# aexoden/snesimage

Hardware: AMD Instinct MI355X
Metric: candidate palettes scored/sec (higher is better)
Workload: dtype f32

## Files before the change

snesimage_amd/csrc/capi.hip:

```cpp
#include "../../include/snesimage_hip.h"
#include "kernels.hpp"
#include "kernels_opt.hpp"
#include "kernels_fast.hpp"
#include "kernels_sparse.hpp"
#include "kernels_sparse2.hpp"
#include "kernels_batch.hpp"
#include "kernels_shared.hpp"
#include "kernels_tile.hpp"

#include <hip/hip_runtime.h>

#include <atomic>
#include <cmath>
#include <cstdio>
#include <cstdlib>
#include <cstring>
#include <string>
#include <utility>
#include <memory>
#include <vector>

using namespace snes;

namespace {
// ... 114 lines not shown
        uint32_t h2q_max = 512;
        bool down_tiles = true;
        uint32_t h0_min = 1024;
        bool base_down_side = false;
        uint32_t h0_grid = 8192;
        hipStream_t h0_stream[8] = {}; hipEvent_t ev_scan[8] = {}, ev_h0[8] = {}, ev_hn[8] = {}, ev_vn[8] = {};
        bool v0_aside = true;
        hipEvent_t ev_v0[8] = {};
        bool vn_aside = true;
        uint32_t tiles_grid = 4096;
        uint32_t down1_grid = 32768;
        bool vsplit = true;
        uint32_t scan4_max = 2048;
        uint32_t hgrid = 8192;
        bool dedup = true; uint32_t dedup_min = 1024; int *holder = nullptr; bool holder_dirty = false;
        bool enabled = false, side = true; uint32_t min_n = 1; uint32_t cap = 0, lanes = 0;
        SparseGeom S{};
        float *store = nullptr, *cand_tab = nullptr, *cand_lab = nullptr, *ckf = nullptr, *ckh = nullptr; long long zeros_off = 0; uint32_t *bitmap = nullptr; double *cka = nullptr, *part = nullptr;
        CandMeta *meta = nullptr; unsigned int *items = nullptr; int *item_count = nullptr; long long item_stride = 0; int *order = nullptr, *first = nullptr;
        uint4 *plist = nullptr; int *plist_count = nullptr; bool plist_valid = false;
        hipStream_t base_stream = nullptr; hipEvent_t ev_base_in = nullptr, ev_base_h = nullptr, ev_base_done = nullptr, ev_base_narrow = nullptr;
        uint8_t *dmaps = nullptr, *dmapsC4 = nullptr;
        uint8_t *bmap = nullptr, *bmapC4 = nullptr, *bcand = nullptr; unsigned long long *dpack = nullptr; double *ckd = nullptr; uint32_t slot_ci = 0;
        float *rec_lab = nullptr;
        int base_sp = -1, base_si = -1;
        struct Ahead { uint8_t *bmap = nullptr, *bmapC4 = nullptr, *bcand = nullptr; unsigned long long *dpack = nullptr; double *ckd = nullptr; float *btab = nullptr, *blab = nullptr, *rec_lab = nullptr; int *ok = nullptr;
                       hipEvent_t ev = nullptr; bool on = true, have = false; int sp = -1, si = -1; unsigned long long epoch = 0; } ahead;
    } sp;
    uint8_t *d_cand = nullptr; uint32_t cand_cap = 0;
    uint8_t *d_cand_sel = nullptr;
// ... 296 lines not shown
    HIPCHK(dmalloc(&sp.store, sizeof(float) * (size_t)S.cand_stride * ncap));
    if (g_poison_alloc.load()) HIPCHK(hipMemsetAsync(sp.store, 0xff, sizeof(float) * (size_t)S.cand_stride * ncap, c->stream));
    HIPCHK(dmalloc(&sp.cand_tab, sizeof(float) * 8 * ncap));
    if (c->perceptual) {
        dfree(sp.cand_lab); dfree(sp.bitmap);
        HIPCHK(dmalloc(&sp.cand_lab, sizeof(float) * 3 * ncap));
        HIPCHK(dmalloc(&sp.bitmap, sizeof(uint32_t) * (c->npx / 32) * ncap));
    }
    HIPCHK(dmalloc(&sp.ckf, sizeof(float) * (size_t)okf));
    dfree(sp.ckh); HIPCHK(dmalloc(&sp.ckh, sizeof(float) * (size_t)(okh + 12LL * G.W + 256)));
    sp.zeros_off = okh;
    HIPCHK(hipMemsetAsync(sp.ckh + okh, 0, sizeof(float) * 12 * (size_t)G.W, c->stream));
    HIPCHK(dmalloc(&sp.cka, sizeof(double) * (size_t)oka));
    HIPCHK(dmalloc(&sp.part, sizeof(double) * ncap * kMaxScales * 18));
    HIPCHK(dmalloc(&sp.meta, sizeof(CandMeta) * ncap));
    dfree(sp.order); HIPCHK(dmalloc(&sp.order, sizeof(int) * ncap));
    dfree(sp.first); HIPCHK(dmalloc(&sp.first, sizeof(int) * ncap));
    HIPCHK(dmalloc(&sp.items, sizeof(unsigned int) * (size_t)sp.item_stride * kItemLists * (c->nlanes + 1)));
    if (!sp.base_stream && sp.side) {
        int prio_lo = 0, prio_hi = 0;
        HIPCHK(hipDeviceGetStreamPriorityRange(&prio_lo, &prio_hi));
        HIPCHK(hipStreamCreateWithPriority(&sp.base_stream, hipStreamNonBlocking, prio_hi));
        HIPCHK(hipEventCreateWithFlags(&sp.ev_base_in, hipEventDisableTiming));
        HIPCHK(hipEventCreateWithFlags(&sp.ev_base_h, hipEventDisableTiming));
        HIPCHK(hipEventCreateWithFlags(&sp.ev_base_narrow, hipEventDisableTiming));
        HIPCHK(hipEventCreateWithFlags(&sp.ev_base_done, hipEventDisableTiming));
    }
    HIPCHK(dmalloc(&sp.item_count, sizeof(int) * (kItemLists * (c->nlanes + 1) + 1)));
    HIPCHK(hipMemsetAsync(sp.item_count, 0, sizeof(int) * (kItemLists * (c->nlanes + 1) + 1), c->stream));
    sp.plist_count = sp.item_count + (size_t)kItemLists * (c->nlanes + 1);
    sp.counters_cleared = true;
// ... 171 lines not shown
        else if (c->ditherw && c->sub_size == 15) hipLaunchKernelGGL((k_ditherw<15>), dim3((nc + 3) / 4), dim3(256), 0, stream, Dp, (int)nc);
        else if (c->ditherw && c->sub_size > 1) hipLaunchKernelGGL((k_ditherw<0>), dim3((nc + 3) / 4), dim3(256), 0, stream, Dp, (int)nc);
        else if (c->sub_size == 15) hipLaunchKernelGGL((k_dither<false, 15, 2>), dim3(nc), dim3(128), 0, stream, Dp);
        else hipLaunchKernelGGL((k_dither<false, 0, 2>), dim3(nc), dim3(128), 0, stream, Dp);
        hipLaunchKernelGGL(k_dither_diff, dim3((nc + 3) / 4), dim3(1024), 0, stream, P);
    } else if (c->perceptual) {
        hipLaunchKernelGGL(k_candidate_lab, dim3((nc + 63) / 64), dim3(64), 0, stream, sp.cand_tab + 8 * (size_t)P.k0, (int)nc, c->d_lab_eotf, sp.cand_lab + 3 * (size_t)P.k0);
        HIPCHK(hipMemsetAsync(sp.bitmap + (size_t)P.k0 * (c->npx / 32), 0, sizeof(uint32_t) * (c->npx / 32) * nc, stream));
        hipLaunchKernelGGL(k_sparse_scan_lab, dim3(nc), dim3(256), 0, stream, P);
    } else if (nc <= sp.scan4_max) hipLaunchKernelGGL(k_sparse_scan4, dim3((nc + 3) / 4), dim3(1024), 0, stream, P);
    else hipLaunchKernelGGL(k_sparse_scan, dim3((nc + 15) / 16), dim3(1024), 0, stream, P);
    bool vn_aside = false;
    const bool h0_ahead = sp.side && sp.h0_min > 0 && nc >= sp.h0_min && nc > sp.h2q_max && lane < 8 && P.s_first > 0;
    const bool v0_aside = h0_ahead && sp.v0_aside;
    vn_aside = h0_ahead && !v0_aside && sp.vn_aside && P.s_first < G.nscales;
    if (c->sp.lpt && nc > 512) P.order = sp.order + P.k0;
    if (h0_ahead) {
        if (!sp.h0_stream[lane]) {
            HIPCHK(hipStreamCreateWithFlags(&sp.h0_stream[lane], hipStreamNonBlocking));
            HIPCHK(hipEventCreateWithFlags(&sp.ev_scan[lane], hipEventDisableTiming));
            HIPCHK(hipEventCreateWithFlags(&sp.ev_h0[lane], hipEventDisableTiming));
            HIPCHK(hipEventCreateWithFlags(&sp.ev_hn[lane], hipEventDisableTiming));
            HIPCHK(hipEventCreateWithFlags(&sp.ev_v0[lane], hipEventDisableTiming));
            HIPCHK(hipEventCreateWithFlags(&sp.ev_vn[lane], hipEventDisableTiming));
        }
        hipStream_t hs = sp.h0_stream[lane];
        HIPCHK(hipEventRecord(sp.ev_scan[lane], stream));
        HIPCHK(hipStreamWaitEvent(hs, sp.ev_scan[lane], 0));
        HIPCHK(hipStreamWaitEvent(hs, sp.ev_base_h, 0));
        size_t gx = ((size_t)nc * (G.sh[0] / 4) * 3 + 15) / 16; if (gx > sp.h0_grid) gx = sp.h0_grid;
        hipLaunchKernelGGL(k_sparse_h2, dim3((unsigned)gx, (unsigned)kColBuckets), dim3(64), h2_lds(c), hs, P);
// ... 34 lines not shown
    if (sp.side || stream != c->stream) HIPCHK(hipStreamWaitEvent(stream, sp.side ? sp.ev_base_done : c->ev_ready, 0));
    if (c->sp.lpt && nc > 512) {
        if (!h0_ahead) hipLaunchKernelGGL(k_sparse_order, dim3(1), dim3(1024), 0, stream, P, sp.order + P.k0);
        P.order = sp.order + P.k0;
    }
    if (vn_aside) {
        hipStream_t hs = sp.h0_stream[lane];
        HIPCHK(hipStreamWaitEvent(hs, sp.ev_hn[lane], 0));
        HIPCHK(hipStreamWaitEvent(hs, sp.ev_base_narrow, 0));
        hipLaunchKernelGGL(k_sparse_v, dim3((nc * 3 + 7) / 8, (unsigned)(G.nscales - P.s_first)), dim3(256), 0, hs, P);
        HIPCHK(hipEventRecord(sp.ev_vn[lane], hs));
    }
    if (v0_aside) {
        if (sp.side) HIPCHK(hipStreamWaitEvent(stream, sp.ev_base_narrow, 0));
        if (P.s_first < G.nscales) hipLaunchKernelGGL(k_sparse_v, dim3((nc * 3 + 7) / 8, (unsigned)(G.nscales - P.s_first)), dim3(256), 0, stream, P);
        if (P.s_first > 1) hipLaunchKernelGGL(k_sparse_v2_from, dim3(nc * 3, (unsigned)(P.s_first - 1)), dim3(256), 0, stream, P, 1);
    } else {
    if (c->timing) HIPCHK(hipEventRecord(tr.ev[3], stream));
    hipLaunchKernelGGL(k_sparse_v2, dim3(nc * 3, (unsigned)P.s_first), dim3(256), 0, stream, P);
    if (c->timing) HIPCHK(hipEventRecord(tr.ev[4], stream));
    }
    if (vn_aside) HIPCHK(hipStreamWaitEvent(stream, sp.ev_vn[lane], 0));
    else if (!v0_aside) {
    if (sp.side) HIPCHK(hipStreamWaitEvent(stream, sp.ev_base_narrow, 0));
    if (P.s_first < G.nscales) hipLaunchKernelGGL(k_sparse_v, dim3((nc * 3 + 7) / 8, (unsigned)(G.nscales - P.s_first)), dim3(256), 0, stream, P);
    }
    if (v0_aside) HIPCHK(hipStreamWaitEvent(stream, sp.ev_v0[lane], 0));
    hipLaunchKernelGGL(k_final_score_wave, dim3((nc + 3) / 4), dim3(256), 0, stream, sp.part + (size_t)P.k0 * G.nscales * 18, (int)nc, G, d_errors, err_stride, err_offset, P.item_count, (int)kItemLists);
    if (c->dither) {
        uint8_t *bm = lane == 0 ? c->d_bestmap : c->extra[lane - 1].d_bestmap; BestRec *br = lane == 0 ? c->d_bestrec : c->extra[lane - 1].d_bestrec;
        hipLaunchKernelGGL(k_keep_best, dim3(1), dim3(1024), 0, stream, d_errors, err_stride, err_offset, (int)nc, P.maps, (int)c->npx, br, bm);
    }
    HIPCHK(hipGetLastError());
    if (c->timing) { tr.light = c->timing != 1; if (!tr.light) HIPCHK(hipEventRecord(tr.ev[5], stream)); c->t_pending.push_back(tr); }
    return SNES_OK;
}

struct LaneScope {
    snesimage_ctx *c; snesimage_ctx::Lane *L;
    LaneScope(snesimage_ctx *c_, snesimage_ctx::Lane *L_) : c(c_), L(L_) { swap(); }
    ~LaneScope() { swap(); }
    void swap() { std::swap(c->stream, L->stream); std::swap(c->d_work, L->d_work); std::swap(c->d_cand_tab, L->d_cand_tab); std::swap(c->d_cand_lab, L->d_cand_lab);
                  std::swap(c->d_part, L->d_part); std::swap(c->d_maps, L->d_maps); std::swap(c->d_mapsT, L->d_mapsT); std::swap(c->d_mapsC4, L->d_mapsC4); std::swap(c->d_mapsR4, L->d_mapsR4);
// ... 212 lines not shown
    if (const char *e = getenv("SNES_DITHER_REC")) c->dither_rec = atoi(e) != 0;
    if (const char *e = getenv("SNES_DITHER4_MAX")) { int v = atoi(e); if (v >= 0) c->dither4_max = (uint32_t)v; }
    if (const char *e = getenv("SNES_DOWN1_GRID")) { int v = atoi(e); if (v >= 64) c->sp.down1_grid = (uint32_t)v; }
    if (const char *e = getenv("SNES_VSPLIT")) c->sp.vsplit = atoi(e) != 0;
    if (const char *e = getenv("SNES_DOWN_TILES")) c->sp.down_tiles = atoi(e) != 0;
    if (const char *e = getenv("SNES_V0_ASIDE")) c->sp.v0_aside = atoi(e) != 0;
    if (const char *e = getenv("SNES_VN_ASIDE")) c->sp.vn_aside = atoi(e) != 0;
    if (const char *e = getenv("SNES_H0_GRID")) { int v = atoi(e); if (v >= 16) c->sp.h0_grid = (uint32_t)v; }
    if (const char *e = getenv("SNES_H0_MIN")) { int v = atoi(e); if (v >= 0) c->sp.h0_min = (uint32_t)v; }
    if (const char *e = getenv("SNES_TILES_GRID")) { int v = atoi(e); if (v >= 64) c->sp.tiles_grid = (uint32_t)v; }
    if (const char *e = getenv("SNES_SCAN4_MAX")) { int v = atoi(e); if (v >= 0) c->sp.scan4_max = (uint32_t)v; }
    if (const char *e = getenv("SNES_H2Q_MAX")) { int v = atoi(e); if (v >= 0) c->sp.h2q_max = (uint32_t)v; }
    if (const char *e = getenv("SNES_HGRID")) { int v = atoi(e); if (v >= 1) c->sp.hgrid = (uint32_t)v; }
    if (const char *e = getenv("SNES_SPARSE_MIN")) { int v = atoi(e); if (v >= 1) c->sp.min_n = (uint32_t)v; }
    if (const char *e = getenv("SNES_DEDUP")) c->sp.dedup = atoi(e) != 0;
    if (const char *e = getenv("SNES_DEDUP_MIN")) { int v = atoi(e); if (v >= 1) c->sp.dedup_min = (uint32_t)v; }
    Geom &G = c->G;
    G.W = (int)w; G.H = (int)h; G.nscales = 0;
    int P2 = 8;
    while (P2 < (int)h) P2 *= 2;
    for (int s = 0; s < kMaxScales; s++) {
        if (s > 0 && (G.sw[s - 1] < 8 || G.th[s - 1] < 8)) break;
        G.sw[s] = (int)w >> s; G.th[s] = s == 0 ? (int)h : (G.th[s - 1] + 1) / 2; G.sh[s] = s == 0 ? (int)h : P2 >> s; G.nscales = s + 1;
    }
    long long off = 0, soff = 0;
    for (int s = 0; s < G.nscales; s++) {
        long long N = (long long)G.sw[s] * G.sh[s];
        G.src_off[s] = soff; soff += 3 * N;
        if (s >= 1) { G.off_xyb[s] = off; off += 3 * N; G.off_xybT[s] = off; off += 3 * N; } else { G.off_xyb[s] = 0; G.off_xybT[s] = 0; }
        G.off_hout[s] = off; off += 9 * N;
// ... 60 lines not shown
}

void batch_forget(struct snesimage_batch *b, snesimage_ctx *c);
void group_forget(struct snesimage_group *g, snesimage_ctx *c);
namespace { void window_free(struct snesimage_window *w); void tile_free(snesimage_ctx *c); }
void snesimage_destroy(snesimage_ctx *c) {
    if (!c) return;
    (void)hipSetDevice(c->device);
    if (c->tile) { if (c->stream) (void)hipStreamSynchronize(c->stream); tile_free(c); }
    if (c->win) { if (c->stream) (void)hipStreamSynchronize(c->stream); window_free(c->win); c->win = nullptr; }
    if (c->owner) batch_forget(c->owner, c);
    if (c->group) group_forget(c->group, c);
    if (c->ev_own) (void)hipEventDestroy(c->ev_own);
    if (c->stream) (void)hipStreamSynchronize(c->stream);
    (void)drain_timing(c);
    dfree(c->d_packC4); dfree(c->d_packR4); dfree(c->d_subC4); dfree(c->d_subR4); dfree(c->d_mapsC4); dfree(c->d_mapsR4); dfree(c->d_img1C4); dfree(c->d_mu1R4); dfree(c->d_sd1R4); dfree(c->d_r1); dfree(c->d_r1R4); dfree(c->d_a1); dfree(c->d_a1R4);
    dfree(c->d_orig); dfree(c->d_tile_pal); dfree(c->d_colors); dfree(c->d_map); dfree(c->d_pack); dfree(c->d_packT); dfree(c->d_eotf); dfree(c->d_lab_eotf);
    dfree(c->d_pal_rgb8); dfree(c->d_pal_lin); dfree(c->d_pal_xyb); dfree(c->d_pal_lab); dfree(c->d_lin0); dfree(c->d_img1); dfree(c->d_img1T); dfree(c->d_mu1); dfree(c->d_sd1);
    dfree(c->d_bestmaps_all); dfree(c->d_bestrecs_all); dfree(c->d_skip); dfree(c->d_rplist); dfree(c->d_rcount); dfree(c->d_rtab); dfree(c->d_rlab); dfree(c->d_tile_cost); dfree(c->d_tile_any); dfree(c->d_tile_moved);
    dfree(c->d_labpx); dfree(c->d_labpxT); dfree(c->d_work); dfree(c->d_cand_tab); dfree(c->d_cand_lab); dfree(c->d_part); dfree(c->d_maps); dfree(c->d_mapsT);
    dfree(c->d_cand); dfree(c->d_cand_sel); dfree(c->d_errs); dfree(c->d_errs_sel); dfree(c->d_inc_err); dfree(c->d_last); dfree(c->d_scratch_err); dfree(c->d_dummy_cand);
    for (auto &L : c->extra) { if (L.stream) (void)hipStreamSynchronize(L.stream); dfree(L.d_mapsC4); dfree(L.d_mapsR4); dfree(L.d_work); dfree(L.d_cand_tab); dfree(L.d_cand_lab); dfree(L.d_part); dfree(L.d_maps); dfree(L.d_mapsT); if (L.done) (void)hipEventDestroy(L.done); if (L.stream) (void)hipStreamDestroy(L.stream); }
    if (c->ev_ready) (void)hipEventDestroy(c->ev_ready);
    { auto &q = c->sp; for (int i = 0; i < 8; i++) if (q.h0_stream[i]) { (void)hipStreamSynchronize(q.h0_stream[i]); (void)hipStreamDestroy(q.h0_stream[i]); (void)hipEventDestroy(q.ev_scan[i]); (void)hipEventDestroy(q.ev_h0[i]); (void)hipEventDestroy(q.ev_hn[i]); (void)hipEventDestroy(q.ev_vn[i]); (void)hipEventDestroy(q.ev_v0[i]); }
      if (q.base_stream) { (void)hipStreamSynchronize(q.base_stream); (void)hipStreamDestroy(q.base_stream); (void)hipEventDestroy(q.ev_base_in); (void)hipEventDestroy(q.ev_base_h); (void)hipEventDestroy(q.ev_base_narrow); (void)hipEventDestroy(q.ev_base_done); } dfree(q.store); dfree(q.cand_tab); dfree(q.ckf); dfree(q.cka); dfree(q.part); dfree(q.meta); dfree(q.items); dfree(q.item_count); dfree(q.plist); dfree(q.order); dfree(q.first); dfree(q.holder); dfree(q.cand_lab); dfree(q.bitmap); dfree(q.ckh);
      dfree(q.dmaps); dfree(q.dmapsC4); dfree(q.bmap); dfree(q.bmapC4); dfree(q.bcand); dfree(q.dpack); dfree(q.ckd);
      dfree(q.rec_lab); dfree(q.ahead.blab); dfree(q.ahead.rec_lab); dfree(q.ahead.bmap); dfree(q.ahead.bmapC4); dfree(q.ahead.bcand); dfree(q.ahead.dpack); dfree(q.ahead.ckd); dfree(q.ahead.btab); dfree(q.ahead.ok); if (q.ahead.ev) (void)hipEventDestroy(q.ahead.ev); }
    kmeans_free(c->km);
    if (c->own_stream) (void)hipStreamDestroy(c->own_stream);
    delete c;
// ... 397 lines not shown
```

snesimage_amd/csrc/kernels.hpp:

```cpp
#pragma once
#include "color.hpp"

namespace snes {

constexpr int kMaxScales = SSIM2_NUM_SCALES;
constexpr int kBlurRadius = 5;

SNES_HD long long idx_c4(int x, int y, int H) { return ((long long)(x >> 2) * H + y) * 4 + (x & 3); }
SNES_HD long long idx_r4(int x, int y, int W) { return ((long long)(y >> 2) * W + x) * 4 + (y & 3); }
SNES_HD long long idx_xt4(int x, int y, int H) { return ((((long long)(x >> 6) * (H >> 2)) + (y >> 2)) << 8) + ((x & 63) << 2) + (y & 3); }

struct BlurK {
    float n2[3];
    float d1[3];
};

struct Geom {
    int W, H, nscales;
    int sw[kMaxScales], sh[kMaxScales];
    int th[kMaxScales];
    long long off_xyb[kMaxScales], off_xybT[kMaxScales], off_hout[kMaxScales];
    long long cand_stride;
    long long src_off[kMaxScales];
};
// ... 647 lines not shown
                ssim = fma(kSsim2Weight[i], fabs(avg_edge[n]), ssim); i++;
                ssim = fma(kSsim2Weight[i], fabs(avg_edge[n + 2]), ssim); i++;
            }
        }
    ssim *= SSIM2_SCORE_SCALE;
    ssim = fma(SSIM2_SCORE_C3 * ssim * ssim, ssim, fma(SSIM2_SCORE_C1, ssim, SSIM2_SCORE_C2 * ssim * ssim));
    if (ssim > 0.0) ssim = fma(pow(ssim, SSIM2_SCORE_EXP), SSIM2_SCORE_GAIN, SSIM2_SCORE_MAX);
    else ssim = SSIM2_SCORE_MAX;
    errors[(size_t)err_offset + (size_t)c * err_stride] = 100.0 - ssim;
}

__device__ __forceinline__ double readlane_f64(double v, int l) {
    const int lo = __builtin_amdgcn_readlane(__double2loint(v), l), hi = __builtin_amdgcn_readlane(__double2hiint(v), l);
    return __hiloint2double(hi, lo);
}
__device__ __forceinline__ void final_score_wave_body(const double *__restrict__ part, int ncand, const Geom &G, double *__restrict__ errors, int err_stride, int err_offset, int *__restrict__ zero, int nzero) {
    const int gt = blockIdx.x * blockDim.x + threadIdx.x;
    if (zero && gt < nzero) zero[gt] = 0;
    const int lane = threadIdx.x & 63, c = __builtin_amdgcn_readfirstlane(gt >> 6);
    if (c >= ncand) return;
    const int ns = G.nscales, npair = 3 * ns;
    double term[6] = {0.0, 0.0, 0.0, 0.0, 0.0, 0.0};
    if (lane < npair) {
        const int ch = lane / ns, s = lane - ch * ns;
        const double *p = part + (((size_t)c * ns + s) * 3 + ch) * 6;
        const double opp = 1.0 / (double)((size_t)G.sw[s] * G.th[s]);
        term[0] = opp * p[0]; term[1] = opp * p[2]; term[2] = opp * p[4];
        term[3] = sqrt(sqrt(opp * p[1])); term[4] = sqrt(sqrt(opp * p[3])); term[5] = sqrt(sqrt(opp * p[5]));
    }
    double ssim = 0.0;
    int i = 0;
    for (int l = 0; l < npair; l++) {
#pragma unroll
        for (int t = 0; t < 6; t++) { ssim = fma(kSsim2Weight[i], fabs(readlane_f64(term[t], l)), ssim); i++; }
    }
    if (lane != 0) return;
    ssim *= SSIM2_SCORE_SCALE;
    ssim = fma(SSIM2_SCORE_C3 * ssim * ssim, ssim, fma(SSIM2_SCORE_C1, ssim, SSIM2_SCORE_C2 * ssim * ssim));
    if (ssim > 0.0) ssim = fma(pow(ssim, SSIM2_SCORE_EXP), SSIM2_SCORE_GAIN, SSIM2_SCORE_MAX);
    else ssim = SSIM2_SCORE_MAX;
    errors[(size_t)err_offset + (size_t)c * err_stride] = 100.0 - ssim;
}

__global__ void k_candidate_tables(const uint8_t *__restrict__ rgb5, int n, const float *__restrict__ eotf, float *__restrict__ cand_tab) { candidate_tables_body(rgb5, n, eotf, cand_tab); }
__global__ void k_candidate_tables_mark(const uint8_t *__restrict__ rgb5, int n, const float *__restrict__ eotf, float *__restrict__ cand_tab, int *__restrict__ holder, int list0) { candidate_tables_mark_body(rgb5, n, eotf, cand_tab, holder, list0); }
__global__ __launch_bounds__(1024) void k_dedup_copy(const uint8_t *__restrict__ rgb5, int n, int *__restrict__ holder, double *__restrict__ errors, int err_stride, int err_offset) { dedup_copy_body(rgb5, n, holder, errors, err_stride, err_offset); }
__global__ __launch_bounds__(256) void k_prep(PrepParams P) { prep_body(P); }
__global__ void k_final_score(const double *__restrict__ part, int ncand, Geom G, double *__restrict__ errors, int err_stride, int err_offset, int *__restrict__ zero = nullptr, int nzero = 0) {
    final_score_body(part, ncand, G, errors, err_stride, err_offset, zero, nzero);
}
__global__ __launch_bounds__(256) void k_final_score_wave(const double *__restrict__ part, int ncand, Geom G, double *__restrict__ errors, int err_stride, int err_offset, int *__restrict__ zero = nullptr, int nzero = 0) {
    final_score_wave_body(part, ncand, G, errors, err_stride, err_offset, zero, nzero);
}

}
```

snesimage_amd/csrc/kernels_sparse.hpp:

```cpp
#pragma once
#include "kernels.hpp"

namespace snes {

constexpr int kGroupsTotal = 126;

struct CandMeta {
    int ngroups[kMaxScales];
    int xmin;
    int won;
    unsigned char glist[kGroupsTotal + 2];
    short gslot[kGroupsTotal];
    unsigned char gcb[kGroupsTotal];
};
__device__ __forceinline__ int item_k(unsigned int it) { return (int)(it >> 14); }
__device__ __forceinline__ int item_g(unsigned int it) { return (int)((it >> 8) & 63u); }
__device__ __forceinline__ int item_j(unsigned int it) { return (int)((it >> 2) & 63u); }
__device__ __forceinline__ int item_ch(unsigned int it) { return (int)(it & 3u); }
constexpr int kColBuckets = 4;
constexpr int kItemLists = kMaxScales * kColBuckets;

struct SparseGeom {
    long long off_lin[kMaxScales], off_xybC[kMaxScales], off_xybR[kMaxScales], off_hout[kMaxScales];
    long long cand_stride;
// ... 8 lines not shown
    const unsigned long long *pack, *packC4, *packR4;
    const uint4 *plist; const int *plist_count;
    const float *pal_lin, *pal_xyb, *cand_tab;
    int perceptual; const float *labpx, *cand_lab; uint32_t *bitmap;
    const float *img1C4, *mu1R4, *sd1R4, *a1R4; const double *r1R4;
    float *store; CandMeta *meta;
    unsigned int *items; int *item_count; long long item_stride;
    float *ckf; double *cka; double *part; float *ckh;
    const float *zeros;
    float *trash;
    int use_maps, sub_size; uint32_t slot_ci; const uint8_t *maps, *mapsC4, *bmap, *bmapC4, *subC4, *tile_pal;
    int s_first;
    int *first;
    const int *order;
    const int *holder; int list0;
};

__device__ __forceinline__ uint32_t sparse_ci(uint32_t lo, uint32_t thr, uint32_t crgb, uint32_t ncol) {
    return red_mean_key(crgb, lo & 0x00ffffffu) < thr ? ncol : (lo >> 24);
}

__device__ __forceinline__ uint32_t won_bit(const uint32_t *bm, int px) { return (bm[px >> 5] >> (px & 31)) & 1u; }
__device__ __forceinline__ uint32_t maps_ci(const SparseParams &P, const uint8_t *map, bool is_base, int x0, int y0, uint32_t pack_lo) {
    uint32_t ci = pack_lo >> 24;
    if (ci != (uint32_t)P.ncol + 1u) {
        ci = (uint32_t)P.tile_pal[(x0 >> 3) + (y0 >> 3) * (P.G.W >> 3)] * (uint32_t)P.sub_size + map[y0 * P.G.W + x0];
        if (!is_base && ci == P.slot_ci) ci = (uint32_t)P.ncol;
    }
    return ci;
}

// ... 852 lines not shown
__device__ __forceinline__ void sparse_v_body(const SparseParams &P, const int s) {
    __shared__ float s_lut[256];
    __shared__ short s_gslot[256];
    __shared__ __attribute__((aligned(16))) unsigned char s_raw[(2 + 3) * 3 * 256 * sizeof(float2)];
    float2 (*s_xy)[3][256] = reinterpret_cast<float2 (*)[3][256]>(s_raw);
    float2 (*s_zw)[3][256] = reinterpret_cast<float2 (*)[3][256]>(s_raw + 2 * 3 * 256 * sizeof(float2));
    double (*red)[6] = reinterpret_cast<double (*)[6]>(s_raw);
    static_assert(sizeof(s_raw) >= 256 * 6 * sizeof(double), "reduction scratch must fit the tail ring");
    const Geom &G = P.G;
    if (s >= G.nscales) return;
    const int W = G.sw[s], H = G.sh[s];
    const bool S0 = S0M == 2 ? s == 0 : S0M == 1;
    const int t = threadIdx.x;
    const int ppw = 256 / W;
    const bool is_base = BM == 2 ? P.is_base != 0 : BM == 1;
    const int npairs = is_base ? 3 : P.ncand * 3;
    if ((int)blockIdx.x * ppw >= npairs) return;
    const int ql = t / W, x = t - ql * W;
    const int pair_raw = blockIdx.x * ppw + ql;
    const bool active = pair_raw < npairs;
    const int pair = active ? pair_raw : 0;
    const int k = is_base ? P.base : P.k0 + (P.order ? P.order[pair / 3] : pair / 3), ch = pair % 3;
    if (S0) {
        s_lut[t] = (t < P.ncol + 2) ? P.pal_xyb[3 * t + ch] : 0.0f;
    }
    const size_t ns = (size_t)W * H;
    const int H4 = H >> 2;
    const CandMeta *M = P.meta + k;
    for (int i = t; i < ppw * H4; i += 256) {
        const int pr = blockIdx.x * ppw + i / H4;
        const int pq = (pr < npairs ? pr : 0) / 3;
// ... 258 lines not shown
            queued -= 64;
            if (lane < queued) { const uint32_t v = q[64 + lane]; q[lane] = v; }
        }
    }
    if (lane < queued) full_test((int)q[lane]);
}

__device__ __forceinline__ void sparse_order_body(const SparseParams &P, int *__restrict__ order) {
    __shared__ int s_cnt[66];
    const int t = threadIdx.x, H4 = P.G.sh[0] >> 2;
    const int *first = P.first + P.k0;
    if (t < 66) s_cnt[t] = 0;
    __syncthreads();
    for (int i = t; i < P.ncand; i += blockDim.x) atomicAdd(&s_cnt[first[i]], 1);
    __syncthreads();
    if (t == 0) { int run = 0; for (int b = 0; b <= H4; b++) { const int c = s_cnt[b]; s_cnt[b] = run; run += c; } }
    __syncthreads();
    for (int i = t; i < P.ncand; i += blockDim.x) order[atomicAdd(&s_cnt[first[i]], 1)] = i;
}
__global__ __launch_bounds__(1024) void k_sparse_order(SparseParams P, int *__restrict__ order) { sparse_order_body(P, order); }

__global__ __launch_bounds__(256) void k_sparse_scan_lab(SparseParams P) { sparse_scan_lab_body(P); }
__global__ __launch_bounds__(1024) void k_sparse_scan(SparseParams P) { sparse_scan_body<1>(P); }
__global__ __launch_bounds__(1024) void k_sparse_scan4(SparseParams P) { sparse_scan_body<4>(P); }
__global__ __launch_bounds__(1024) void k_dither_first(SparseParams P) { dither_first_body(P); }
__global__ __launch_bounds__(256) void k_dither_first_lab(SparseParams P) { dither_first_lab_body(P); }
__global__ __launch_bounds__(1024) void k_dither_diff(SparseParams P) { dither_diff_body(P); }
__global__ __launch_bounds__(256) void k_sparse_down(SparseParams P, int only_scale) { sparse_down_body(P, only_scale, (int)blockIdx.x); }
__global__ __launch_bounds__(256) void k_sparse_down1(SparseParams P) { sparse_down1_body(P, (int)blockIdx.x, (int)gridDim.x); }
__global__ __launch_bounds__(256) void k_sparse_down_tiles(SparseParams P) { sparse_down_tiles_body<SNES_DOWN_TILES_U>(P, (int)blockIdx.x, (int)gridDim.x); }
__global__ __launch_bounds__(256) void k_base_down(SparseParams P) { base_down_body(P); }
// ... 6 lines not shown
```

snesimage_amd/csrc/kernels_sparse2.hpp:

```cpp
#pragma once
#include "kernels_sparse.hpp"
#include "kernels_fast.hpp"

namespace snes {

#define SNES_HSTEP(SUM, A, B, OUT)                                                   \
    {                                                                                \
        float o1_ = (SUM) * n2_0, o3_ = (SUM) * n2_1, o5_ = (SUM) * n2_2;            \
        o1_ = fmaf(-1.0f, B[0], o1_); o3_ = fmaf(-1.0f, B[1], o3_); o5_ = fmaf(-1.0f, B[2], o5_); \
        o1_ = fmaf(mp_0, A[0], o1_); o3_ = fmaf(mp_1, A[1], o3_); o5_ = fmaf(mp_2, A[2], o5_);    \
        B[0] = o1_; B[1] = o3_; B[2] = o5_;                                          \
        OUT = o1_ + o3_ + o5_;                                                       \
    }
#define SNES_VSTEP(SUM, A, B, OUT)                                                   \
    {                                                                                \
        float o1_ = fmaf(A[0], d1_0, B[0]), o3_ = fmaf(A[1], d1_1, B[1]), o5_ = fmaf(A[2], d1_2, B[2]); \
        o1_ = fmaf((SUM), n2_0, -o1_); o3_ = fmaf((SUM), n2_1, -o3_); o5_ = fmaf((SUM), n2_2, -o5_);    \
        B[0] = o1_; B[1] = o3_; B[2] = o5_;                                          \
        OUT = o1_ + o3_ + o5_;                                                       \
    }

struct H2Shared {
    __attribute__((aligned(16))) float out[16 * (4 * 32 + 4)];
    long long hbase[16], xbase[16];
// ... 325 lines not shown
    const u32x4 v = __builtin_amdgcn_raw_buffer_load_b128(r, (int)voff, (int)soff, 0);
    return make_double2(__hiloint2double((int)v.y, (int)v.x), __hiloint2double((int)v.w, (int)v.z));
}

template <bool BASE>
__device__ __forceinline__ void sparse_v2_body(const SparseParams &P, const int s, const int bx) {
    __shared__ short s_slot[4][64];
    __shared__ __attribute__((aligned(16))) unsigned char s_raw[(2 + 3) * 3 * 256 * sizeof(float2)];
    double (*red)[6] = reinterpret_cast<double (*)[6]>(s_raw);
    static_assert(sizeof(s_raw) >= 256 * 6 * sizeof(double), "reduction scratch must fit the tail ring");
    const Geom &G = P.G;
    const int W = uni(G.sw[s]), H = uni(G.sh[s]), H4 = H >> 2;
    const int t = threadIdx.x, lane = t & 63;
    const int wv = uni(t >> 6);
    const int wpp = W >> 6, ppw = 4 / wpp;
    const int npairs = BASE ? 3 : P.ncand * 3;
    if (bx * ppw >= npairs) return;
    const int ql = wv / wpp, xw = (wv - ql * wpp) << 6;
    const int pair_raw = bx * ppw + ql;
    const bool active = pair_raw < npairs;
    const int pair = active ? pair_raw : 0;
    const int ch = BASE ? pair : pair / P.ncand, ci = BASE ? 0 : pair - ch * P.ncand;
    const int k = BASE ? P.base : uni(P.k0 + (P.order ? P.order[ci] : ci));
    const CandMeta *M = P.meta + k;
    int gs;
    {
        const int g = lane;
        short sl = -1;
        if (!BASE && g < H4) { sl = M->gslot[P.S.goff[s] + g]; if (sl >= 0 && ((int)M->gcb[P.S.goff[s] + g] << 6) > xw) sl = -1; }
        s_slot[wv][lane] = sl;
        const unsigned long long own = __ballot(sl >= 0);
        gs = BASE ? 0 : uni(own ? __ffsll((long long)own) - 1 : H4 + 1);
    }
    __syncthreads();

    const size_t ns = (size_t)W * H;
    const float *store_k = P.store + (size_t)k * P.S.cand_stride, *store_b = P.store + (size_t)P.base * P.S.cand_stride;
// ... 235 lines not shown

template <bool BASE>
__device__ __forceinline__ void sparse_h2_dispatch(const SparseParams &P, const int list, const int bx, const int gx) {
    const int s = list / kColBuckets;
    if (s >= P.G.nscales || P.G.sw[s] < 64 || (list % kColBuckets) >= (P.G.sw[s] >> 6)) return;
    __shared__ H2Shared sh;
    if (s == 0) sparse_h2_body<true, BASE>(P, list, bx, gx, sh); else sparse_h2_body<false, BASE>(P, list, bx, gx, sh);
}
__global__ __launch_bounds__(64) void k_sparse_h2(SparseParams P) { sparse_h2_dispatch<false>(P, (int)blockIdx.y, (int)blockIdx.x, (int)gridDim.x); }
__global__ __launch_bounds__(64) void k_sparse_h2_from(SparseParams P, int list0) { sparse_h2_dispatch<false>(P, list0 + (int)blockIdx.y, (int)blockIdx.x, (int)gridDim.x); }
__global__ __launch_bounds__(64) void k_sparse_h2q(SparseParams P) { sparse_h2q_dispatch<false>(P, (int)blockIdx.y, (int)blockIdx.x, (int)gridDim.x); }
__global__ __launch_bounds__(64) void k_sparse_h2q_base(SparseParams P) { sparse_h2q_dispatch<true>(P, (int)blockIdx.y, (int)blockIdx.x, (int)gridDim.x); }
__global__ __launch_bounds__(64) void k_sparse_h2_base(SparseParams P) { sparse_h2_dispatch<true>(P, (int)blockIdx.y, (int)blockIdx.x, (int)gridDim.x); }
__global__ __launch_bounds__(256, 5) void k_sparse_v2(SparseParams P) { if ((int)blockIdx.y < P.G.nscales && P.G.sw[blockIdx.y] >= 64) sparse_v2_body<false>(P, (int)blockIdx.y, (int)blockIdx.x); }
__global__ __launch_bounds__(256, 5) void k_sparse_v2_from(SparseParams P, int s0) { const int s = s0 + (int)blockIdx.y; if (s < P.G.nscales && P.G.sw[s] >= 64) sparse_v2_body<false>(P, s, (int)blockIdx.x); }
__global__ __launch_bounds__(128) void k_sparse_v2_base_split(SparseParams P) { const int s = (int)blockIdx.z; if (s < P.G.nscales && P.G.sw[s] >= 64 && (int)blockIdx.x < (P.G.sw[s] >> 6)) sparse_v2_base_split_body(P, s, (int)blockIdx.y, (int)blockIdx.x); }
__global__ __launch_bounds__(256) void k_sparse_v2_base(SparseParams P) { if ((int)blockIdx.y < P.G.nscales && P.G.sw[blockIdx.y] >= 64) sparse_v2_body<true>(P, (int)blockIdx.y, (int)blockIdx.x); }
__device__ __forceinline__ void sparse_v_base_narrow_dispatch(const SparseParams &P) { const int s = (int)blockIdx.y + P.s_first; if (s < P.G.nscales) sparse_v_body<false, 0, 1>(P, s); }
__global__ __launch_bounds__(256, 1) void k_sparse_v_base_narrow(SparseParams P) { sparse_v_base_narrow_dispatch(P); }

}
```

Before: 2.846 million.

## Skip scoring of empty candidates and flatten v2 launch across scales

The LPT ordering kernel now records how many candidates touch any pixels (n_live). The vertical sparse kernels then only process that many candidates plus one representative empty one, and the final scoring kernel copies the representative empty candidate's score to every empty candidate in order. The multi-scale v2 launch is also flattened into a single 1D grid sized to exact per-scale block counts, which removes dead blocks for wider scales. This relies on empty candidates all having an identical score equal to one shared representative. It adds an indirection and an optional synchronous counting path.

```diff
diff --git a/profiles/empty_share.py b/profiles/empty_share.py
--- /dev/null
+++ b/profiles/empty_share.py
@@ -0,0 +1,66 @@
+#!/usr/bin/env python3
+import argparse
+import os
+import sys
+
+import numpy as np
+
+sys.path.insert(0, os.path.dirname(os.path.dirname(os.path.abspath(__file__))))
+
+
+def expand5(v):
+    v = np.asarray(v, np.int64)
+    return (v * 8 + v // 4) & 0xff
+
+
+def key(c, p):
+    dr, dg, db = c[..., 0] - p[..., 0], c[..., 1] - p[..., 1], c[..., 2] - p[..., 2]
+    rs = c[..., 0] + p[..., 0]
+    return (1024 + rs) * dr * dr + 2048 * dg * dg + (1534 - rs) * db * db
+
+
+def main():
+    ap = argparse.ArgumentParser()
+    ap.add_argument("--slots", type=int, default=64)
+    ap.add_argument("--n", type=int, default=4096)
+    ap.add_argument("--seed", type=int, default=1)
+    ap.add_argument("--first", type=int, default=10, help="step id of the first call (the benchmark's timed calls start at 10)")
+    a = ap.parse_args()
+    from oracle import oracle_py as O
+    from snesimage_amd import schedule
+    from snesimage_amd.synth import synth_image
+
+    img = synth_image()
+    o = O.OracleImage(img, 8, 15)
+    o.initialize_tiles()
+    o.recalculate_palettes()
+    tp, pal = np.asarray(o.tile_palettes), expand5(np.asarray(o.palette))
+    H = img.shape[0]
+    sub_of_px = np.repeat(np.repeat(tp[:(H // 8) * 32].reshape(H // 8, 32), 8, axis=0), 8, axis=1)
+    opaque = img[..., 3] != 0
+    rows = []
+    for i, (_, sp, si, _, _) in enumerate(schedule(8, 15, a.first + a.slots)[a.first:]):
+        px = np.unique(img[(sub_of_px == sp) & opaque][:, :3].astype(np.int64), axis=0)
+        others = [j for j in range(15) if j != si]
+        k_o = key(pal[sp * 15 + np.array(others)][:, None, :], px[None, :, :])
+        best = np.argmin(k_o, axis=0)
+        thr = k_o[best, np.arange(px.shape[0])] + (si < np.array(others)[best])
+        cand = np.asarray(O.random_candidates(a.seed, a.first + i, a.n)).reshape(-1, 3)
+        c8 = expand5(cand)
+        wins = np.zeros(a.n, bool)
+        for c0 in range(0, a.n, 512):
+            wins[c0:c0 + 512] = (key(c8[c0:c0 + 512, None, :], px[None, :, :]) < thr[None, :]).any(axis=1)
+        k15 = cand[:, 0].astype(np.int64) | (cand[:, 1].astype(np.int64) << 5) | (cand[:, 2].astype(np.int64) << 10)
+        firsts = np.zeros(a.n, bool)
+        firsts[np.unique(k15, return_index=True)[1]] = True
+        rows.append((sp, si, int((~wins).sum()), int((~firsts).sum()), int((~(wins & firsts)).sum())))
+    r = np.array(rows)
+    print("| slots | candidates per call | win no pixel | duplicates | empty for the scan (either) | min..max of the last by slot |")
+    print("|---|---|---|---|---|---|")
+    print("| %d | %d | %.1f %% | %.1f %% | %.1f %% | %.1f %% .. %.1f %% |" % (
+        len(rows), a.n, 100.0 * r[:, 2].mean() / a.n, 100.0 * r[:, 3].mean() / a.n, 100.0 * r[:, 4].mean() / a.n,
+        100.0 * r[:, 4].min() / a.n, 100.0 * r[:, 4].max() / a.n))
+
+
+if __name__ == "__main__":
+    main()
diff --git a/snesimage_amd/csrc/capi.hip b/snesimage_amd/csrc/capi.hip
--- a/snesimage_amd/csrc/capi.hip
+++ b/snesimage_amd/csrc/capi.hip
@@ -152,6 +152,8 @@
         uint32_t scan4_max = 2048;
         uint32_t hgrid = 8192;
         bool dedup = true; uint32_t dedup_min = 1024; int *holder = nullptr; bool holder_dirty = false;
+        bool skip_empty = true; int *n_live = nullptr;
+        bool count_empty = false; unsigned long long ce_cands = 0, ce_empty = 0;
         bool enabled = false, side = true; uint32_t min_n = 1; uint32_t cap = 0, lanes = 0;
         SparseGeom S{};
         float *store = nullptr, *cand_tab = nullptr, *cand_lab = nullptr, *ckf = nullptr, *ckh = nullptr; long long zeros_off = 0; uint32_t *bitmap = nullptr; double *cka = nullptr, *part = nullptr;
@@ -478,7 +480,7 @@
     HIPCHK(dmalloc(&sp.cka, sizeof(double) * (size_t)oka));
     HIPCHK(dmalloc(&sp.part, sizeof(double) * ncap * kMaxScales * 18));
     HIPCHK(dmalloc(&sp.meta, sizeof(CandMeta) * ncap));
-    dfree(sp.order); HIPCHK(dmalloc(&sp.order, sizeof(int) * ncap));
+    dfree(sp.order); HIPCHK(dmalloc(&sp.order, sizeof(int) * (ncap + lanes))); sp.n_live = sp.order + ncap;
     dfree(sp.first); HIPCHK(dmalloc(&sp.first, sizeof(int) * ncap));
     HIPCHK(dmalloc(&sp.items, sizeof(unsigned int) * (size_t)sp.item_stride * kItemLists * (c->nlanes + 1)));
     if (!sp.base_stream && sp.side) {
@@ -680,7 +682,9 @@
     const bool h0_ahead = sp.side && sp.h0_min > 0 && nc >= sp.h0_min && nc > sp.h2q_max && lane < 8 && P.s_first > 0;
     const bool v0_aside = h0_ahead && sp.v0_aside;
     vn_aside = h0_ahead && !v0_aside && sp.vn_aside && P.s_first < G.nscales;
+    const bool skip_empty = sp.skip_empty && c->sp.lpt && nc > 512 && !c->dither;
     if (c->sp.lpt && nc > 512) P.order = sp.order + P.k0;
+    if (skip_empty) P.n_live = sp.n_live + lane;
     if (h0_ahead) {
         if (!sp.h0_stream[lane]) {
             HIPCHK(hipStreamCreateWithFlags(&sp.h0_stream[lane], hipStreamNonBlocking));
@@ -745,6 +749,8 @@
     if (v0_aside) {
         if (sp.side) HIPCHK(hipStreamWaitEvent(stream, sp.ev_base_narrow, 0));
         if (P.s_first < G.nscales) hipLaunchKernelGGL(k_sparse_v, dim3((nc * 3 + 7) / 8, (unsigned)(G.nscales - P.s_first)), dim3(256), 0, stream, P);
+        if (P.s_first > 1 && skip_empty) { unsigned nb = 0; for (int s = 1; s < P.s_first; s++) nb += (unsigned)sparse_v2_blocks(G, (int)nc, s); hipLaunchKernelGGL(k_sparse_v2_flat, dim3(nb), dim3(256), 0, stream, P, 1); }
+        else
         if (P.s_first > 1) hipLaunchKernelGGL(k_sparse_v2_from, dim3(nc * 3, (unsigned)(P.s_first - 1)), dim3(256), 0, stream, P, 1);
     } else {
     if (c->timing) HIPCHK(hipEventRecord(tr.ev[3], stream));
@@ -757,7 +763,13 @@
     if (P.s_first < G.nscales) hipLaunchKernelGGL(k_sparse_v, dim3((nc * 3 + 7) / 8, (unsigned)(G.nscales - P.s_first)), dim3(256), 0, stream, P);
     }
     if (v0_aside) HIPCHK(hipStreamWaitEvent(stream, sp.ev_v0[lane], 0));
-    hipLaunchKernelGGL(k_final_score_wave, dim3((nc + 3) / 4), dim3(256), 0, stream, sp.part + (size_t)P.k0 * G.nscales * 18, (int)nc, G, d_errors, err_stride, err_offset, P.item_count, (int)kItemLists);
+    hipLaunchKernelGGL(k_final_score_wave, dim3((nc + 3) / 4), dim3(256), 0, stream, sp.part + (size_t)P.k0 * G.nscales * 18, (int)nc, G, d_errors, err_stride, err_offset, P.item_count, (int)kItemLists, P.n_live ? P.order : nullptr, P.n_live);
+    if (sp.count_empty && P.n_live) {
+        int live = 0;
+        HIPCHK(hipStreamSynchronize(stream));
+        HIPCHK(hipMemcpy(&live, P.n_live, sizeof(int), hipMemcpyDeviceToHost));
+        sp.ce_cands += nc; sp.ce_empty += nc - (uint32_t)live;
+    }
     if (c->dither) {
         uint8_t *bm = lane == 0 ? c->d_bestmap : c->extra[lane - 1].d_bestmap; BestRec *br = lane == 0 ? c->d_bestrec : c->extra[lane - 1].d_bestrec;
         hipLaunchKernelGGL(k_keep_best, dim3(1), dim3(1024), 0, stream, d_errors, err_stride, err_offset, (int)nc, P.maps, (int)c->npx, br, bm);
@@ -1000,6 +1012,8 @@
     if (const char *e = getenv("SNES_HGRID")) { int v = atoi(e); if (v >= 1) c->sp.hgrid = (uint32_t)v; }
     if (const char *e = getenv("SNES_SPARSE_MIN")) { int v = atoi(e); if (v >= 1) c->sp.min_n = (uint32_t)v; }
     if (const char *e = getenv("SNES_DEDUP")) c->sp.dedup = atoi(e) != 0;
+    if (const char *e = getenv("SNES_SKIP_EMPTY")) c->sp.skip_empty = atoi(e) != 0;
+    if (const char *e = getenv("SNES_COUNT_EMPTY")) c->sp.count_empty = atoi(e) != 0;
     if (const char *e = getenv("SNES_DEDUP_MIN")) { int v = atoi(e); if (v >= 1) c->sp.dedup_min = (uint32_t)v; }
     Geom &G = c->G;
     G.W = (int)w; G.H = (int)h; G.nscales = 0;
@@ -1090,6 +1104,7 @@
     if (c->ev_own) (void)hipEventDestroy(c->ev_own);
     if (c->stream) (void)hipStreamSynchronize(c->stream);
     (void)drain_timing(c);
+    if (c->sp.count_empty && c->sp.ce_cands) fprintf(stderr, "snesimage: %llu of %llu candidates were empty (SNES_COUNT_EMPTY)\n", c->sp.ce_empty, c->sp.ce_cands);
     dfree(c->d_packC4); dfree(c->d_packR4); dfree(c->d_subC4); dfree(c->d_subR4); dfree(c->d_mapsC4); dfree(c->d_mapsR4); dfree(c->d_img1C4); dfree(c->d_mu1R4); dfree(c->d_sd1R4); dfree(c->d_r1); dfree(c->d_r1R4); dfree(c->d_a1); dfree(c->d_a1R4);
     dfree(c->d_orig); dfree(c->d_tile_pal); dfree(c->d_colors); dfree(c->d_map); dfree(c->d_pack); dfree(c->d_packT); dfree(c->d_eotf); dfree(c->d_lab_eotf);
     dfree(c->d_pal_rgb8); dfree(c->d_pal_lin); dfree(c->d_pal_xyb); dfree(c->d_pal_lab); dfree(c->d_lin0); dfree(c->d_img1); dfree(c->d_img1T); dfree(c->d_mu1); dfree(c->d_sd1);
diff --git a/snesimage_amd/csrc/kernels.hpp b/snesimage_amd/csrc/kernels.hpp
--- a/snesimage_amd/csrc/kernels.hpp
+++ b/snesimage_amd/csrc/kernels.hpp
@@ -685,11 +685,14 @@
     const int lo = __builtin_amdgcn_readlane(__double2loint(v), l), hi = __builtin_amdgcn_readlane(__double2hiint(v), l);
     return __hiloint2double(hi, lo);
 }
-__device__ __forceinline__ void final_score_wave_body(const double *__restrict__ part, int ncand, const Geom &G, double *__restrict__ errors, int err_stride, int err_offset, int *__restrict__ zero, int nzero) {
+__device__ __forceinline__ void final_score_wave_body(const double *__restrict__ part, int ncand, const Geom &G, double *__restrict__ errors, int err_stride, int err_offset, int *__restrict__ zero, int nzero,
+                                                      const int *__restrict__ order = nullptr, const int *__restrict__ n_live = nullptr) {
     const int gt = blockIdx.x * blockDim.x + threadIdx.x;
     if (zero && gt < nzero) zero[gt] = 0;
-    const int lane = threadIdx.x & 63, c = __builtin_amdgcn_readfirstlane(gt >> 6);
-    if (c >= ncand) return;
+    const int lane = threadIdx.x & 63, w = __builtin_amdgcn_readfirstlane(gt >> 6);
+    if (w >= ncand) return;
+    const int c_out = n_live ? __builtin_amdgcn_readfirstlane(order[w]) : w;
+    const int c = n_live ? __builtin_amdgcn_readfirstlane(order[min(w, *n_live)]) : w;
     const int ns = G.nscales, npair = 3 * ns;
     double term[6] = {0.0, 0.0, 0.0, 0.0, 0.0, 0.0};
     if (lane < npair) {
@@ -710,7 +713,7 @@
     ssim = fma(SSIM2_SCORE_C3 * ssim * ssim, ssim, fma(SSIM2_SCORE_C1, ssim, SSIM2_SCORE_C2 * ssim * ssim));
     if (ssim > 0.0) ssim = fma(pow(ssim, SSIM2_SCORE_EXP), SSIM2_SCORE_GAIN, SSIM2_SCORE_MAX);
     else ssim = SSIM2_SCORE_MAX;
-    errors[(size_t)err_offset + (size_t)c * err_stride] = 100.0 - ssim;
+    errors[(size_t)err_offset + (size_t)c_out * err_stride] = 100.0 - ssim;
 }
 
 __global__ void k_candidate_tables(const uint8_t *__restrict__ rgb5, int n, const float *__restrict__ eotf, float *__restrict__ cand_tab) { candidate_tables_body(rgb5, n, eotf, cand_tab); }
@@ -720,8 +723,9 @@
 __global__ void k_final_score(const double *__restrict__ part, int ncand, Geom G, double *__restrict__ errors, int err_stride, int err_offset, int *__restrict__ zero = nullptr, int nzero = 0) {
     final_score_body(part, ncand, G, errors, err_stride, err_offset, zero, nzero);
 }
-__global__ __launch_bounds__(256) void k_final_score_wave(const double *__restrict__ part, int ncand, Geom G, double *__restrict__ errors, int err_stride, int err_offset, int *__restrict__ zero = nullptr, int nzero = 0) {
-    final_score_wave_body(part, ncand, G, errors, err_stride, err_offset, zero, nzero);
-}
-
-}
+__global__ __launch_bounds__(256) void k_final_score_wave(const double *__restrict__ part, int ncand, Geom G, double *__restrict__ errors, int err_stride, int err_offset, int *__restrict__ zero = nullptr, int nzero = 0,
+                                                          const int *__restrict__ order = nullptr, const int *__restrict__ n_live = nullptr) {
+    final_score_wave_body(part, ncand, G, errors, err_stride, err_offset, zero, nzero, order, n_live);
+}
+
+}
diff --git a/snesimage_amd/csrc/kernels_sparse.hpp b/snesimage_amd/csrc/kernels_sparse.hpp
--- a/snesimage_amd/csrc/kernels_sparse.hpp
+++ b/snesimage_amd/csrc/kernels_sparse.hpp
@@ -46,7 +46,9 @@
     int *first;
     const int *order;
     const int *holder; int list0;
+    int *n_live;
 };
+__device__ __forceinline__ int sparse_dealt(const SparseParams &P) { return P.n_live ? min(P.ncand, *P.n_live + 1) : P.ncand; }
 
 __device__ __forceinline__ uint32_t sparse_ci(uint32_t lo, uint32_t thr, uint32_t crgb, uint32_t ncol) {
     return red_mean_key(crgb, lo & 0x00ffffffu) < thr ? ncol : (lo >> 24);
@@ -929,7 +931,7 @@
     const int t = threadIdx.x;
     const int ppw = 256 / W;
     const bool is_base = BM == 2 ? P.is_base != 0 : BM == 1;
-    const int npairs = is_base ? 3 : P.ncand * 3;
+    const int npairs = is_base ? 3 : sparse_dealt(P) * 3;
     if ((int)blockIdx.x * ppw >= npairs) return;
     const int ql = t / W, x = t - ql * W;
     const int pair_raw = blockIdx.x * ppw + ql;
@@ -1218,7 +1220,7 @@
     __syncthreads();
     for (int i = t; i < P.ncand; i += blockDim.x) atomicAdd(&s_cnt[first[i]], 1);
     __syncthreads();
-    if (t == 0) { int run = 0; for (int b = 0; b <= H4; b++) { const int c = s_cnt[b]; s_cnt[b] = run; run += c; } }
+    if (t == 0) { int run = 0; for (int b = 0; b <= H4; b++) { const int c = s_cnt[b]; s_cnt[b] = run; run += c; } if (P.n_live) *P.n_live = s_cnt[H4]; }
     __syncthreads();
     for (int i = t; i < P.ncand; i += blockDim.x) order[atomicAdd(&s_cnt[first[i]], 1)] = i;
 }
diff --git a/snesimage_amd/csrc/kernels_sparse2.hpp b/snesimage_amd/csrc/kernels_sparse2.hpp
--- a/snesimage_amd/csrc/kernels_sparse2.hpp
+++ b/snesimage_amd/csrc/kernels_sparse2.hpp
@@ -363,13 +363,14 @@
     const int t = threadIdx.x, lane = t & 63;
     const int wv = uni(t >> 6);
     const int wpp = W >> 6, ppw = 4 / wpp;
-    const int npairs = BASE ? 3 : P.ncand * 3;
+    const int nd = BASE ? 1 : uni(sparse_dealt(P));
+    const int npairs = nd * 3;
     if (bx * ppw >= npairs) return;
     const int ql = wv / wpp, xw = (wv - ql * wpp) << 6;
     const int pair_raw = bx * ppw + ql;
     const bool active = pair_raw < npairs;
     const int pair = active ? pair_raw : 0;
-    const int ch = BASE ? pair : pair / P.ncand, ci = BASE ? 0 : pair - ch * P.ncand;
+    const int ch = BASE ? pair : pair / nd, ci = BASE ? 0 : pair - ch * nd;
     const int k = BASE ? P.base : uni(P.k0 + (P.order ? P.order[ci] : ci));
     const CandMeta *M = P.meta + k;
     int gs;
@@ -635,6 +636,12 @@
 __global__ __launch_bounds__(64) void k_sparse_h2_base(SparseParams P) { sparse_h2_dispatch<true>(P, (int)blockIdx.y, (int)blockIdx.x, (int)gridDim.x); }
 __global__ __launch_bounds__(256, 5) void k_sparse_v2(SparseParams P) { if ((int)blockIdx.y < P.G.nscales && P.G.sw[blockIdx.y] >= 64) sparse_v2_body<false>(P, (int)blockIdx.y, (int)blockIdx.x); }
 __global__ __launch_bounds__(256, 5) void k_sparse_v2_from(SparseParams P, int s0) { const int s = s0 + (int)blockIdx.y; if (s < P.G.nscales && P.G.sw[s] >= 64) sparse_v2_body<false>(P, s, (int)blockIdx.x); }
+__host__ __device__ __forceinline__ int sparse_v2_blocks(const Geom &G, int ncand, int s) { const int ppb = 4 / (G.sw[s] >> 6); return (ncand * 3 + ppb - 1) / ppb; }
+__global__ __launch_bounds__(256, 5) void k_sparse_v2_flat(SparseParams P, int s0) {
+    int s = s0, b = (int)blockIdx.x;
+    for (; s < P.s_first; s++) { const int nb = sparse_v2_blocks(P.G, P.ncand, s); if (b < nb) break; b -= nb; }
+    if (s < P.s_first) sparse_v2_body<false>(P, s, b);
+}
 __global__ __launch_bounds__(128) void k_sparse_v2_base_split(SparseParams P) { const int s = (int)blockIdx.z; if (s < P.G.nscales && P.G.sw[s] >= 64 && (int)blockIdx.x < (P.G.sw[s] >> 6)) sparse_v2_base_split_body(P, s, (int)blockIdx.y, (int)blockIdx.x); }
 __global__ __launch_bounds__(256) void k_sparse_v2_base(SparseParams P) { if ((int)blockIdx.y < P.G.nscales && P.G.sw[blockIdx.y] >= 64) sparse_v2_body<true>(P, (int)blockIdx.y, (int)blockIdx.x); }
 __device__ __forceinline__ void sparse_v_base_narrow_dispatch(const SparseParams &P) { const int s = (int)blockIdx.y + P.s_first; if (s < P.G.nscales) sparse_v_body<false, 0, 1>(P, s); }
```

Result: faster. 2.878 million, median of 6 (+1.1%).
